# scroll-tech/halo2-snark-aggregator

Measured on AMD Instinct MI355X. Metric: BN254 G1 MSM points/sec, higher is better.
Workload: dtype u32 (9 x 29-bit limbs, Montgomery R = 2^261; 254-bit prime-field integers)

## Files before the change

halo2-snark-aggregator_amd/__init__.py:

```python
from __future__ import annotations

import ctypes as C
import os
from typing import List, Optional, Sequence

_HERE = os.path.dirname(os.path.abspath(__file__))
LIB_PATH = os.path.join(_HERE, "libh2agg.so")
HEADER_PATH = os.path.join(os.path.dirname(_HERE), "include", "h2agg.h")

OK, ERR_INVALID, ERR_DIV_ZERO, ERR_EMPTY, ERR_HIP, ERR_NONCANONICAL, ERR_NOMEM, ERR_BAD_POINT, ERR_PEER, ERR_NOT_IN_TABLE = range(10)
OP_ADD, OP_SUB, OP_MUL, OP_SQR, OP_INV, OP_DIV = range(6)
FR_FFT_LOCAL = 10
FR_FFT_MAX_K = 24
FR_QUOTIENT_MAX_K = 28
LAUNCH_ELEMENTWISE = (8, 256)
LAUNCH_SCALAR_MUL = (16, 32)
LAUNCH_SIZE_ORDER = (4, 256)
LAUNCH_MSM_FIX = (12, 64)
LAUNCH_MSM_BIG = (8, 64)
FR_POLY_CHUNK = 11
FR_SCAN_CHUNK = 11
FR_PROD_MAX_COLUMNS = 16
FR_SORT_TILE = 11
FR_SORT_TILE_MIN = 4
# ... 69 lines not shown
        "h2agg_host_alloc": (i32, [ctxp, sz, C.POINTER(vp)]),
        "h2agg_host_free": (i32, [ctxp, vp]),
        "h2agg_eval_flat": (i32, [ctxp, u8p, u8p, u8p, sz, vp]),
        "h2agg_bases_upload": (i32, [ctxp, u8p, sz, C.POINTER(u64)]),
        "h2agg_bases_generate": (i32, [ctxp, vp, sz, C.POINTER(u64)]),
        "h2agg_bases_precompute": (i32, [ctxp, u64, i32]),
        "h2agg_bases_download": (i32, [ctxp, u64, sz, sz, vp]),
        "h2agg_bases_free": (i32, [ctxp, u64]),
        "h2agg_g1_msm_preloaded": (i32, [ctxp, u64, u8p, sz, vp]),
        "h2agg_instance_commitment": (i32, [ctxp, u64, u8p, sz, sz, vp]),
        "h2agg_g1_msm_device": (i32, [ctxp, u64, vp, sz, vp]),
        "h2agg_g1_msm_device_async": (i32, [ctxp, u64, vp, sz, vp]),
        "h2agg_schema_create": (i32, [ctxp, C.POINTER(C.c_void_p)]),
        "h2agg_schema_destroy": (None, [C.c_void_p]),
        "h2agg_schema_node_commitment": (i32, [C.c_void_p, C.c_char_p, u8p, C.POINTER(C.c_uint32)]),
        "h2agg_schema_node_eval": (i32, [C.c_void_p, u8p, C.POINTER(C.c_uint32)]),
        "h2agg_schema_node_scalar": (i32, [C.c_void_p, u8p, C.POINTER(C.c_uint32)]),
        "h2agg_schema_node_add": (i32, [C.c_void_p, C.c_uint32, C.c_uint32, C.POINTER(C.c_uint32)]),
        "h2agg_schema_node_mul": (i32, [C.c_void_p, C.c_uint32, C.c_uint32, C.POINTER(C.c_uint32)]),
        "h2agg_schema_estimate": (i32, [C.c_void_p, C.c_uint32, C.POINTER(C.c_size_t)]),
        "h2agg_schema_evaluation_queries": (i32, [C.c_void_p, sz, C.POINTER(C.c_char_p), u8p, u8p,
                                                  C.POINTER(C.c_uint32)]),
        "h2agg_schema_batch_multi_open": (i32, [C.c_void_p, C.c_char_p, sz, C.POINTER(C.c_int32), u8p,
                                                C.POINTER(C.c_uint32), sz, u8p, u8p, u8p,
                                                C.POINTER(C.c_uint32), C.POINTER(C.c_uint32)]),
        "h2agg_schema_shplonk_multi_open": (i32, [C.c_void_p, C.c_char_p, sz, C.POINTER(C.c_uint32), C.POINTER(C.c_int32), u8p,
                                                  C.POINTER(C.c_uint32), u8p, u8p, u8p, u8p, u8p,
                                                  C.POINTER(C.c_uint32), C.POINTER(C.c_uint32)]),
        "h2agg_schema_eval": (i32, [C.c_void_p, C.c_uint32, vp, C.POINTER(i32), vp]),
        "h2agg_evaluate_multiopen_proof": (i32, [C.c_void_p, C.c_uint32, C.c_uint32, vp, vp]),
        "h2agg_evaluate_multiopen_prepare": (i32, [C.c_void_p, C.c_uint32, C.c_uint32]),
        "h2agg_schema_name_count": (C.c_size_t, [C.c_void_p]),
        "h2agg_schema_name": (C.c_char_p, [C.c_void_p, C.c_size_t]),
        "h2agg_g1_msm_device_batch_async": (C.c_int, [C.c_void_p, C.c_uint64, C.c_void_p, C.c_size_t, C.c_size_t, C.c_void_p]),
        "h2agg_schema_query_set_commitment": (C.c_int, [C.c_void_p, C.c_uint32, C.c_char_p]),
        "h2agg_g1_batch_to_affine_device": (C.c_int, [C.c_void_p, C.c_void_p, C.c_size_t, C.c_char_p]),
        "h2agg_schema_names_joined": (C.c_size_t, [C.c_void_p, C.c_char_p, C.c_size_t]),
        "h2agg_schema_point_list_len": (C.c_size_t, [C.c_void_p]),
        "h2agg_poseidon_squeeze_batch": (i32, [ctxp, u8p, sz, sz, C.POINTER(C.c_uint32), sz, vp]),
        "h2agg_transcript_read_batch": (i32, [ctxp, u8p, sz, sz, C.c_char_p, sz, u8p, sz, u8p, sz, vp, vp]),
        "h2agg_vk_create": (i32, [ctxp, u8p, sz, C.POINTER(C.c_void_p)]),
        "h2agg_vk_set_transcript": (i32, [C.c_void_p, i32]),
        "h2agg_vk_set_multiopen": (i32, [C.c_void_p, i32]),
        "h2agg_hash_transcript_read_batch": (i32, [ctxp, i32, u8p, sz, sz, C.c_char_p, sz, u8p, sz, u8p, sz, vp, vp]),
        "h2agg_hash_transcript_read_batch_host": (i32, [i32, u8p, sz, sz, C.c_char_p, sz, u8p, sz, u8p, sz, vp, vp, i32]),
        "h2agg_hash_digest_host": (i32, [i32, u8p, sz, vp]),
        "h2agg_vk_destroy": (None, [C.c_void_p]),
        "h2agg_verify_aggregation": (i32, [ctxp, vp, sz, u8p, u8p, vp, vp, vp, C.POINTER(i32)]),
        "h2agg_verify_aggregation_ex": (i32, [ctxp, vp, sz, u8p, u8p, vp, vp, vp, C.POINTER(i32), vp, sz]),
        "h2agg_verify_aggregation_sharded": (i32, [ctxp, vp, sz, vp, u8p, u8p, vp, vp, vp, C.POINTER(i32), vp, sz]),
        "h2agg_debug_configure": (i32, [ctxp, C.c_char_p, i32]),
        "h2agg_debug_lean_variant": (i32, [i32, i32]),
        "h2agg_debug_table_identity": (i32, [ctxp, u64, C.POINTER(i32), C.POINTER(i32)]),
        "h2agg_verify_proofs": (i32, [ctxp, vp, sz, u8p, u8p, vp, vp, C.POINTER(C.c_int32), C.POINTER(i32), vp, sz]),
        "h2agg_verify_plan_stats": (i32, [ctxp, C.POINTER(C.c_uint64), C.POINTER(C.c_uint64), C.POINTER(C.c_uint64)]),
        "h2agg_last_phases": (C.c_char_p, [ctxp]),
        "h2agg_transcript_configure": (i32, [ctxp, i32]),
        "h2agg_poseidon_squeeze_batch_host": (i32, [u8p, sz, sz, C.POINTER(C.c_uint32), sz, vp, i32]),
        "h2agg_host_threads": (i32, []),
        "h2agg_host_sponge_kind": (i32, []),
        "h2agg_comm_unique_id": (i32, [vp]),
        "h2agg_comm_init_rank": (i32, [ctxp, u8p, i32, i32]),
        "h2agg_comm_create": (i32, [C.POINTER(i32), i32, C.POINTER(ctxp)]),
        "h2agg_comm_size": (i32, [ctxp]),
        "h2agg_comm_rank": (i32, [ctxp]),
        "h2agg_comm_last_error": (C.c_char_p, []),
        "h2agg_allgather_add_points": (i32, [C.POINTER(ctxp), i32, u8p, sz, vp]),
        "h2agg_pairing_check": (i32, [ctxp, u8p, u8p, sz, C.POINTER(i32)]),
        "h2agg_g2_batch_decompress": (i32, [ctxp, u8p, sz, vp]),
        "h2agg_bases_fft": (i32, [ctxp, u64, C.c_uint, i32, C.POINTER(u64)]),
        "h2agg_params_setup": (i32, [ctxp, C.c_uint, u8p, C.POINTER(u64), C.POINTER(u64)]),
        "h2agg_fr_fft": (i32, [ctxp, vp, C.c_uint, i32, u8p, vp]),
        "h2agg_fr_fft_device": (i32, [ctxp, vp, C.c_uint, i32, u8p, vp]),
        "h2agg_fr_fft_batch": (i32, [ctxp, vp, C.c_size_t, C.c_uint, i32, u8p, vp]),
        "h2agg_fr_poly_eval": (i32, [ctxp, vp, sz, C.c_uint, C.POINTER(C.c_uint32), sz, u8p, sz, vp]),
        "h2agg_fr_poly_eval_device": (i32, [ctxp, vp, sz, C.c_uint, C.POINTER(C.c_uint32), sz, u8p, sz, vp]),
        "h2agg_fr_poly_divide": (i32, [ctxp, vp, C.c_uint, u8p, vp, vp]),
        "h2agg_fr_poly_divide_device": (i32, [ctxp, vp, C.c_uint, u8p, vp, vp]),
        "h2agg_kzg_multiopen": (i32, [ctxp, u64, vp, sz, C.c_uint, C.POINTER(C.c_uint32), sz, u8p, sz, u8p, vp,
                                      C.POINTER(C.c_uint32), C.POINTER(sz)]),
        "h2agg_kzg_multiopen_device": (i32, [ctxp, u64, vp, sz, C.c_uint, C.POINTER(C.c_uint32), sz, u8p, sz, u8p, vp,
                                             C.POINTER(C.c_uint32), C.POINTER(sz)]),
        "h2agg_kzg_shplonk_begin": (i32, [ctxp, u64, vp, sz, C.c_uint, C.POINTER(C.c_uint32), sz, u8p, sz, u8p, u8p, u8p, vp,
                                          C.POINTER(vp)]),
        "h2agg_kzg_shplonk_finish": (i32, [vp, u8p, vp]),
        "h2agg_kzg_shplonk_destroy": (None, [vp]),
        "h2agg_fr_batch_invert": (i32, [ctxp, vp, sz, vp]),
        "h2agg_fr_batch_invert_device": (i32, [ctxp, vp, sz, vp]),
        "h2agg_fr_grand_product": (i32, [ctxp, vp, vp, C.c_uint, sz, u8p, vp, vp]),
        "h2agg_fr_grand_product_device": (i32, [ctxp, vp, vp, C.c_uint, sz, u8p, vp, vp]),
        "h2agg_permutation_product": (i32, [ctxp, vp, vp, sz, C.c_uint, sz, u8p, u8p, u8p, u8p, u8p, vp, vp]),
        "h2agg_permutation_product_device": (i32, [ctxp, vp, vp, sz, C.c_uint, sz, u8p, u8p, u8p, u8p, u8p, vp, vp]),
        "h2agg_lookup_product": (i32, [ctxp, vp, vp, vp, vp, C.c_uint, sz, u8p, u8p, vp, vp]),
        "h2agg_lookup_product_device": (i32, [ctxp, vp, vp, vp, vp, C.c_uint, sz, u8p, u8p, vp, vp]),
        "h2agg_lookup_permute": (i32, [ctxp, vp, vp, C.c_uint, sz, vp, vp]),
        "h2agg_lookup_permute_device": (i32, [ctxp, vp, vp, C.c_uint, sz, vp, vp]),
        "h2agg_lookup_batch_permute": (i32, [ctxp, vp, vp, sz, C.c_uint, sz, vp, vp, vp]),
        "h2agg_lookup_batch_product": (i32, [ctxp, vp, vp, vp, vp, sz, C.c_uint, sz, u8p, u8p, vp, vp]),
        "h2agg_lookup_store_permute": (i32, [ctxp, u64, sz, u64, sz, sz, sz, u64, sz, u64, sz, vp]),
        "h2agg_lookup_store_product": (i32, [ctxp, u64, sz, u64, sz, u64, sz, u64, sz, sz, sz, u8p, u8p, u64, sz, vp]),
        "h2agg_lookup_configure": (i32, [ctxp, sz]),
        "h2agg_lookup_chunk_rule": (sz, [sz, sz]),
        "h2agg_fr_columns_compress": (i32, [ctxp, vp, sz, C.c_uint, u8p, vp]),
        "h2agg_fr_columns_compress_device": (i32, [ctxp, vp, sz, C.c_uint, u8p, vp]),
        "h2agg_vk_expressions_eval": (i32, [ctxp, vp, i32, sz, C.c_uint, vp, vp, vp, u8p, u8p, vp]),
        "h2agg_vk_expressions_eval_device": (i32, [ctxp, vp, i32, sz, C.c_uint, vp, vp, vp, u8p, u8p, vp]),
# ... 969 lines not shown
        _need(g2_aff, 128 * n, "g2_aff")
        ok = C.c_int()
        self._check(self._lib.h2agg_pairing_check(self._ctx, g1_aff, g2_aff, n, C.byref(ok)))
        return bool(ok.value)

    def pairing_product(self, g1_aff: bytes, g2_aff: bytes) -> bytes:
        n = len(g1_aff) // 64
        _need(g1_aff, 64 * n, "g1_aff")
        _need(g2_aff, 128 * n, "g2_aff")
        out = C.create_string_buffer(384)
        self._check(self._lib.h2agg_pairing_product(self._ctx, g1_aff, g2_aff, n, out))
        return out.raw

    def g2_batch_decompress(self, data: bytes) -> bytes:
        n = len(data) // 64
        _need(data, 64 * n, "data")
        out = C.create_string_buffer(max(128 * n, 1))
        self._check(self._lib.h2agg_g2_batch_decompress(self._ctx, data, n, out))
        return out.raw[:128 * n]

    def final_pair_check(self, left_aff: bytes, right_aff: bytes, s_g2: bytes, g2: bytes) -> bool:
        _need(left_aff, 64, "left_aff")
        _need(right_aff, 64, "right_aff")
        _need(s_g2, 128, "s_g2")
        _need(g2, 128, "g2")
        ok = C.c_int()
        self._check(self._lib.h2agg_final_pair_check(self._ctx, left_aff, right_aff, s_g2, g2, C.byref(ok)))
        return bool(ok.value)

    def g1_msm_device_batch_async(self, handle: int, d_scalars_ptr: int, n: int, batch: int, d_out_ptr: int):
        self._check(self._lib.h2agg_g1_msm_device_batch_async(self._ctx, handle, C.c_void_p(d_scalars_ptr), n, batch,
                                                              C.c_void_p(d_out_ptr)))

    def msm_configure(self, window_bits: int = 0, reduce_segment: int = 0, big_bucket_threshold: int = 0):
        self._check(self._lib.h2agg_msm_configure(self._ctx, window_bits, reduce_segment, big_bucket_threshold))

    def msm_configure_glv(self, mode: int = 0):
        self._check(self._lib.h2agg_msm_configure_glv(self._ctx, mode))

    def msm_configure_lanes_per_bucket(self, lanes: int = 0):
        self._check(self._lib.h2agg_msm_configure_lanes_per_bucket(self._ctx, lanes))

    def msm_configure_sort(self, sub_bits: int = 0, tile: int = 0):
        self._check(self._lib.h2agg_msm_configure_sort(self._ctx, sub_bits, tile))

    def debug_configure(self, key: str, value: int):
        self._check(self._lib.h2agg_debug_configure(self._ctx, key.encode(), int(value)))

    def table_may_hold_identity(self, handle: int) -> bool:
        v = C.c_int32(-1)
        self._check(self._lib.h2agg_debug_table_identity(self._ctx, handle, C.byref(v), None))
        return bool(v.value)

    def last_lean_variant(self) -> int:
        v = C.c_int32(-1)
        self._check(self._lib.h2agg_debug_table_identity(self._ctx, 0, None, C.byref(v)))
        return v.value

    def msm_set_tail_overlap(self, level: int = 2):
        self._check(self._lib.h2agg_msm_set_tail_overlap(self._ctx, int(level)))

    def profile_enable(self, on=True, only_stage: Optional[int] = None):
        mode = (2 + int(only_stage)) if (on and only_stage is not None) else int(bool(on))
        self._check(self._lib.h2agg_profile_enable(self._ctx, mode))

    def profile_reset(self):
        self._check(self._lib.h2agg_profile_reset(self._ctx))

    def profile_stages(self):
        out = {}
        for i in range(self._lib.h2agg_profile_stage_count(self._ctx)):
            ms, cnt = C.c_double(), C.c_uint64()
            self._check(self._lib.h2agg_profile_stage_get(self._ctx, i, C.byref(ms), C.byref(cnt)))
            out[self._lib.h2agg_profile_stage_name(self._ctx, i).decode()] = (ms.value, cnt.value)
        return out


def host_sponge_kind() -> str:
    return "ifma" if load_library().h2agg_host_sponge_kind() == 1 else "scalar"


def poseidon_squeeze_batch_host(elems: bytes, nproofs: int, upto: Sequence[int], max_threads: int = 0,
                                kernel: Optional[str] = None) -> bytes:
    lib = load_library()
    max_threads = (max_threads & 0xffff) | {None: 0, "scalar": 0x10000, "ifma": 0x20000}[kernel]
    nelem = (len(elems) // 32) // max(nproofs, 1)
    _need(elems, 32 * nelem * nproofs, "elems")
    nsq = len(upto)
    arr = (C.c_uint32 * max(nsq, 1))(*upto)
    out = C.create_string_buffer(32 * max(nproofs * nsq, 1))
    rc = lib.h2agg_poseidon_squeeze_batch_host(elems, nproofs, nelem, arr, nsq, out, max_threads)
    if rc != OK:
        raise H2AggError(rc, "h2agg_poseidon_squeeze_batch_host: " + ("element >= r" if rc == ERR_NONCANONICAL else "invalid arguments"))
    return out.raw[:32 * nproofs * nsq]


TRANSCRIPT_KINDS = {"poseidon": 0, "sha256": 1, "keccak256": 2}


def _hash_transcript_args(kind, proofs, script, consts, ext_points_aff):
    nproofs = len(proofs)
    plen = 64 * script.count("P") + 32 * script.count("S")
    for p in proofs:
        _need(p, plen, "proof")
    npts, nsq, nx = script.count("P"), script.count("Q"), script.count("X")
    _need(consts, 32 * script.count("C"), "consts")
# ... 213 lines not shown
```

halo2-snark-aggregator_amd/csrc/config_api.inc:

```

namespace {

struct DebugKey {
    const char* name;
    int h2agg_ctx::*field;
    int lo = 1, hi = 0;
    bool zero_ok = false;
};
const DebugKey DEBUG_KEYS[] = {
    {"pcie_slices", &h2agg_ctx::dbg_pcie_slices},
    {"pcie_glv", &h2agg_ctx::dbg_pcie_glv},
    {"pcie_chain", &h2agg_ctx::dbg_pcie_chain},
    {"comb_msm", &h2agg_ctx::dbg_comb_msm},
    {"plan_cache", &h2agg_ctx::dbg_plan_cache},
    {"small_sort", &h2agg_ctx::dbg_small_sort},
    {"eval_split", &h2agg_ctx::dbg_eval_split},
    {"lean_acc", &h2agg_ctx::dbg_lean_acc},
    {"lean_full", &h2agg_ctx::dbg_lean_full},
    {"pre_big", &h2agg_ctx::dbg_pre_big},
    {"tape_lds", &h2agg_ctx::dbg_tape_lds},
    {"prewake", &h2agg_ctx::dbg_prewake},
    {"phases", &h2agg_ctx::dbg_phases},
    {"shard_fail", &h2agg_ctx::dbg_shard_fail},
    {"seg_chunk", &h2agg_ctx::dbg_seg_chunk},
// ... 43 lines not shown
    if (!c) return H2AGG_ERR_INVALID;
    if (lanes != 0 && lanes != 1 && lanes != 2 && lanes != 4 && lanes != 8 && lanes != 16)
        return fail(c, H2AGG_ERR_INVALID, "lanes must be 0, 1, 2, 4, 8 or 16");
    c->cfg_lpb = lanes;
    return H2AGG_OK;
} API_CATCH

int h2agg_msm_configure_sort(h2agg_ctx* c, int sub_bits, int tile) try {
    if (!c) return H2AGG_ERR_INVALID;
    if (sub_bits != 0 && (sub_bits < 4 || sub_bits > SORT_MAX_SUB_BITS))
        return fail(c, H2AGG_ERR_INVALID, "sub_bits must be 0 or in [4, 12]");
    if (tile != 0 && tile != -1 && tile != -2 && tile != -3 && (tile < BLOCK || tile > (1 << 16)))
        return fail(c, H2AGG_ERR_INVALID, "tile must be 0, -1, -2 or in [256, 65536]");
    c->cfg_sub_bits = sub_bits;
    c->cfg_no_stage = tile == -1;
    c->cfg_no_dm = tile == -3;
    c->cfg_stage_l1 = tile == -2;
    c->cfg_tile = tile > 0 ? tile : 0;
    return H2AGG_OK;
} API_CATCH

int h2agg_debug_configure(h2agg_ctx* c, const char* key, int value) try {
    if (!c || !key) return H2AGG_ERR_INVALID;
    const std::string k(key);
    const DebugKey* row = nullptr;
    for (const DebugKey& r : DEBUG_KEYS)
        if (k == r.name) row = &r;
    if (!row) return fail(c, H2AGG_ERR_INVALID, "h2agg_debug_configure: unknown key " + k);
    if (!debug_key_takes(*row, value)) return fail(c, H2AGG_ERR_INVALID, debug_key_range(*row));
#ifndef H2AGG_MEASURE_KNOBS
    if (k == "lean_acc" && value != 1)
        return fail(c, H2AGG_ERR_INVALID, "h2agg_debug_configure: the generic accumulation kernel is in the measure build only (build_ext.py --measure)");
#endif
    if (k == "tape_lds" && c->dbg_tape_lds != value) agg_plans_release(c);
    c->*(row->field) = value;
    return H2AGG_OK;
} API_CATCH

int h2agg_debug_lean_variant(int table_no_identity, int plan_glv) {
    return msm_lean_variant(table_no_identity != 0, plan_glv != 0);
}

int h2agg_debug_table_identity(h2agg_ctx* c, uint64_t handle, int* may_hold_out, int* last_variant_out) try {
    TRY(bind(c));
    if (may_hold_out) {
        Table* t = nullptr;
        TRY(find_table(c, handle, &t));
        *may_hold_out = t->no_identity ? 0 : 1;
    }
    if (last_variant_out) *last_variant_out = c->last_lean_variant;
    return H2AGG_OK;
} API_CATCH

int h2agg_msm_set_tail_overlap(h2agg_ctx* c, int enable) try {
    TRY(bind(c));
    TRY(join_tails(c));
    HIP_TRY(c, hipStreamSynchronize(c->stream));
    c->tail_overlap = enable != 0;
    if (enable >= 1 && enable <= 3) c->overlap_level = enable;
    return H2AGG_OK;
} API_CATCH

int h2agg_profile_enable(h2agg_ctx* c, int enable) try {
    TRY(bind(c));
    if (enable && !c->prof_events_created) {
        for (int r = 0; r < h2agg_ctx::PROF_RING; ++r)
            for (int s = 0; s < ST_N; ++s)
                for (int k = 0; k < 2; ++k) HIP_TRY(c, c->prof[r].ev[s][k].create(EV_TIME_FLAGS));
        c->prof_events_created = true;
    }
    if (!enable) profile_harvest_all(c);
    c->profiling = enable != 0;
    c->prof_only = (enable >= 2 && enable - 2 < ST_N) ? enable - 2 : -1;
    return H2AGG_OK;
} API_CATCH
int h2agg_profile_reset(h2agg_ctx* c) try {
    if (!c) return H2AGG_ERR_INVALID;
    profile_harvest_all(c);
    for (int s = 0; s < ST_N; ++s) {
        c->stage_ms[s] = 0;
        c->stage_launches[s] = 0;
    }
    return H2AGG_OK;
} API_CATCH
int h2agg_profile_stage_count(h2agg_ctx*) { return ST_N; }
const char* h2agg_profile_stage_name(h2agg_ctx*, int i) { return (i >= 0 && i < ST_N) ? STAGE_NAMES[i] : ""; }
int h2agg_profile_stage_get(h2agg_ctx* c, int i, double* total_ms, uint64_t* launches) try {
    if (!c || i < 0 || i >= ST_N) return H2AGG_ERR_INVALID;
    profile_harvest_all(c);
    if (total_ms) *total_ms = c->stage_ms[i];
    if (launches) *launches = c->stage_launches[i];
    return H2AGG_OK;
} API_CATCH

}
```

halo2-snark-aggregator_amd/csrc/sort_kernels.hpp:

```cpp
#pragma once
#include "batch_kernels.hpp"

namespace h2agg {

#ifndef H2AGG_NO_SORT_SETPRIO
#define SORT_PRIO() __builtin_amdgcn_s_setprio(3)
#else
#define SORT_PRIO() ((void)0)
#endif

constexpr int SORT_MAX_PW = 2048;
constexpr int SORT_SUB_BITS = 9;
constexpr int SORT_MAX_SUB_BITS = 12;
constexpr int SORT_MAX_SB = 1 << SORT_MAX_SUB_BITS;
constexpr int SIZE_BINS = 1024;

struct SortPlan {
    int sub_bits;
    uint32_t SB;
    uint32_t ppw;
    uint32_t PW;
    uint32_t tile;
    bool glv;
    uint32_t n_base = 0;
// ... 797 lines not shown
    return x;
}
FP_INLINE void dm_block_scan(uint32_t* v, uint32_t cnt) {
    __syncthreads();
    if (threadIdx.x < 64) {
        const uint32_t lane = threadIdx.x;
        uint32_t x[8], sum = 0;
#pragma unroll
        for (int j = 0; j < 8; ++j) {
            x[j] = (8 * lane + j < cnt) ? v[8 * lane + j] : 0u;
            sum += x[j];
        }
        const uint32_t inc = dm_wave_scan_incl(sum, lane);
        uint32_t off = inc - sum;
#pragma unroll
        for (int j = 0; j < 8; ++j) {
            if (8 * lane + j < cnt) v[8 * lane + j] = off;
            off += x[j];
        }
        if (lane == 63) v[cnt] = inc;
    }
    __syncthreads();
}

__global__ void __launch_bounds__(1024) k_dm_scan(const uint32_t* __restrict__ in, uint32_t n, uint32_t* __restrict__ out) {
    SORT_PRIO();
    __shared__ uint32_t wsum[16];
    const uint32_t tid = threadIdx.x, lane = tid & 63, wave = tid >> 6;
    uint32_t x[8], sum = 0;
#pragma unroll
    for (int j = 0; j < 8; ++j) {
        x[j] = (8 * tid + j < n) ? in[8 * tid + j] : 0u;
        sum += x[j];
    }
    const uint32_t inc = dm_wave_scan_incl(sum, lane);
    if (lane == 63) wsum[wave] = inc;
    __syncthreads();
    uint32_t base = 0;
    for (uint32_t k = 0; k < wave; ++k) base += wsum[k];
    uint32_t off = base + inc - sum;
#pragma unroll
    for (int j = 0; j < 8; ++j) {
        if (8 * tid + j <= n) out[8 * tid + j] = off;
        off += x[j];
    }
    if (8 * tid + 8 == n) out[n] = off;
}

template <bool WIDE>
__global__ void __launch_bounds__(DM_TB1) k_dm_partition(const uint16_t* __restrict__ codes, DmPlan dp,
                                                         uint32_t* __restrict__ pcount, uint32_t* __restrict__ toff,
                                                         uint32_t* __restrict__ items) {
    SORT_PRIO();
    __shared__ uint32_t cnt[DM_MAX_PPW + 1];
    __shared__ __attribute__((aligned(16))) uint32_t stage[DM_T1];
    const uint32_t tile = blockIdx.x, w = blockIdx.y;
    const int tid = threadIdx.x;
    for (uint32_t p = tid; p <= dp.ppw; p += DM_TB1) cnt[p] = 0;
    __syncthreads();
    const size_t row = (size_t)w * dp.n_pad;
    const uint32_t t0 = tile * DM_T1;
    constexpr int G = 8, NV = DM_PER1 / G;
    uint4 v[NV];
    uint32_t sg[NV], zr[NV];
#pragma unroll
    for (int k = 0; k < NV; ++k) {
        const uint32_t i0 = t0 + (k * DM_TB1 + tid) * G;
        sg[k] = 0;
        zr[k] = 0xffu;
        if (WIDE) {
            v[k] = make_uint4(0, 0, 0, 0);
            if (i0 < dp.n_pad) {
                const uint8_t* fl = dm17_flags(codes, dp.n_pad);
                const size_t rb = dp.n_pad >> 3;
                v[k] = *reinterpret_cast<const uint4*>(codes + row + i0);
                sg[k] = fl[(size_t)w * rb + (i0 >> 3)];
                zr[k] = fl[(size_t)(DM17_W + w) * rb + (i0 >> 3)];
            }
        } else {
            v[k] = (i0 < dp.n_pad) ? *reinterpret_cast<const uint4*>(codes + row + i0)
                                   : make_uint4(0x80008000u, 0x80008000u, 0x80008000u, 0x80008000u);
        }
    }
    auto decode = [&](int k, int e, uint32_t& bkt, uint32_t& neg) -> bool {
        const uint32_t wd[4] = {v[k].x, v[k].y, v[k].z, v[k].w};
        const uint32_t code = (wd[e >> 1] >> (16 * (e & 1))) & 0xffffu;
        if (WIDE) {
            bkt = code;
            neg = (sg[k] >> e) & 1u;
            return !((zr[k] >> e) & 1u);
        }
        neg = code >> 15;
        bkt = neg ? (code & 0x7fffu) - 1u : code;
        return code != DM_ZERO;
    };
    uint32_t pr[DM_PER1];
    const uint32_t submask = dp.SB - 1u;
#pragma unroll
    for (int k = 0; k < NV; ++k) {
#pragma unroll
        for (int e = 0; e < G; ++e) {
            uint32_t bkt, neg;
            const uint32_t i = t0 + (k * DM_TB1 + tid) * G + e;
            const bool ok = decode(k, e, bkt, neg) && i < dp.n;
            const uint32_t p = bkt >> dp.sub_bits;
            pr[k * G + e] = ok ? ((p << 16) | atomicAdd(&cnt[p], 1u)) : 0xffffffffu;
        }
    }
    __syncthreads();
    for (uint32_t p = tid; p < dp.ppw; p += DM_TB1) {
        const uint32_t c = cnt[p];
        if (c) atomicAdd(&pcount[w * dp.ppw + p], c);
    }
    dm_block_scan(cnt, dp.ppw);
    uint32_t* tt = toff + ((size_t)w * dp.ntile + tile) * (dp.ppw + 1);
    for (uint32_t p = tid; p <= dp.ppw; p += DM_TB1) tt[p] = cnt[p];
#pragma unroll
    for (int k = 0; k < NV; ++k) {
#pragma unroll
        for (int e = 0; e < G; ++e) {
            const uint32_t q = pr[k * G + e];
            if (q == 0xffffffffu) continue;
            uint32_t bkt, neg;
            decode(k, e, bkt, neg);
            const uint32_t i = t0 + (k * DM_TB1 + tid) * G + e;
            stage[cnt[q >> 16] + (q & 0xffffu)] = ((bkt & submask) << (dp.idx_bits + 1)) | (neg << dp.idx_bits) | i;
        }
    }
    __syncthreads();
    const uint32_t total = cnt[dp.ppw];
    uint32_t* out = items + (size_t)w * dp.n_row + t0;
    for (uint32_t k = 4 * tid; k < total; k += 4 * DM_TB1)
        *reinterpret_cast<uint4*>(out + k) = *reinterpret_cast<const uint4*>(stage + k);
}

FP_INLINE uint32_t dm_entry(uint32_t it, const DmPlan& dp, uint32_t idxmask) {
    uint32_t idx = it & idxmask;
    uint32_t e = ((it >> dp.idx_bits) & 1u) << 31;
    if (idx >= dp.n_pts) {
        idx -= dp.n_pts;
        e |= ENT_ENDO;
    }
    return e | idx;
}

typedef __attribute__((address_space(3))) uint32_t lds_u32;
FP_INLINE uint32_t dm_wave_agg_add(lds_u32* h, uint32_t b, bool valid) {
    const uint32_t lane = __lane_id();
    uint64_t todo = __ballot(valid);
    uint32_t res = 0;
    bool pending = valid;
#pragma unroll 1
    for (int round = 0; round < 2 && todo; ++round) {
        const int lead = __ffsll((unsigned long long)todo) - 1;
        const uint32_t bl = __shfl(b, lead);
        const bool mine = pending && b == bl;
        const uint64_t same = __ballot(mine);
        uint32_t base = 0;
        if ((int)lane == lead)
            base = __hip_atomic_fetch_add(&h[bl], (uint32_t)__popcll(same), __ATOMIC_RELAXED, __HIP_MEMORY_SCOPE_WORKGROUP);
        base = __shfl(base, lead);
        if (mine) {
            res = base + (uint32_t)__popcll(same & ((1ull << lane) - 1ull));
            pending = false;
        }
        todo &= ~same;
    }
    if (pending) res = __hip_atomic_fetch_add(&h[b], 1u, __ATOMIC_RELAXED, __HIP_MEMORY_SCOPE_WORKGROUP);
    return res;
}

template <bool PLACE>
__device__ __attribute__((noinline)) void dm_long_pass(const uint32_t* __restrict__ rowp, const lds_u32* rstart,
                                                       const lds_u32* rpre, lds_u32* h, uint32_t* __restrict__ out,
                                                       uint32_t ntile, int idx_bits, uint32_t n_pts) {
    constexpr int LB = 8;
    const uint32_t lane = threadIdx.x & 63u, wv = threadIdx.x >> 6;
    const int sh = idx_bits + 1;
    const uint32_t idxmask = (1u << idx_bits) - 1u;
    for (uint32_t t = wv; t < ntile; t += DM_TB2 / 64) {
        const uint32_t len = rpre[t + 1] - rpre[t];
        const uint32_t* src = rowp + (size_t)t * DM_T1 + rstart[t];
        for (uint32_t k0 = 0; k0 < len; k0 += 64 * LB) {
            uint32_t v[LB];
#pragma unroll
            for (int j = 0; j < LB; ++j) {
                const uint32_t k = k0 + j * 64 + lane;
                v[j] = k < len ? src[k] : 0u;
            }
#pragma unroll
            for (int j = 0; j < LB; ++j) {
                const bool ok = k0 + j * 64 + lane < len;
                const uint32_t at = dm_wave_agg_add(h, v[j] >> sh, ok);
                if (PLACE && ok) {
                    uint32_t idx = v[j] & idxmask, e = ((v[j] >> idx_bits) & 1u) << 31;
                    if (idx >= n_pts) {
                        idx -= n_pts;
                        e |= ENT_ENDO;
                    }
                    out[at] = e | idx;
                }
            }
        }
    }
}

template <int PER>
__global__ void __launch_bounds__(DM_TB2) __attribute__((amdgpu_waves_per_eu(6, 6))) k_dm_bucket_sort(const uint32_t* __restrict__ pstart,
                                                           const uint32_t* __restrict__ toff,
                                                           const uint32_t* __restrict__ items, DmPlan dp, uint32_t NB,
                                                           uint32_t* __restrict__ hist, uint32_t* __restrict__ offs,
                                                           uint32_t* __restrict__ entries) {
    SORT_PRIO();
    constexpr int TB = DM_TB2;
    __shared__ uint32_t h[DM_MAX_PPW + 8];
    __shared__ uint32_t rstart[DM_MAX_TILES];
    __shared__ uint32_t rpre[DM_MAX_TILES + 8];
    constexpr int DM_STAGE = PER * DM_TB2;
    __shared__ __attribute__((aligned(16))) uint32_t stage[DM_STAGE];
    const uint32_t p = gridDim.x - 1u - blockIdx.x, w = p / dp.ppw, pl = p - w * dp.ppw;
    const int tid = threadIdx.x;
    const uint32_t start = pstart[p], total = pstart[p + 1] - start;
    for (uint32_t b = tid; b <= dp.SB; b += TB) h[b] = 0;
    for (uint32_t t = tid; t < dp.ntile; t += TB) {
        const uint32_t* tt = toff + ((size_t)w * dp.ntile + t) * (dp.ppw + 1) + pl;
        const uint32_t a = tt[0];
        rstart[t] = a;
        rpre[t] = tt[1] - a;
    }
    dm_block_scan(rpre, dp.ntile);
    const uint32_t* rowp = items + (size_t)w * dp.n_row;
    const int sh = dp.idx_bits + 1;
    const uint32_t idxmask = (1u << dp.idx_bits) - 1u;
    const uint32_t key0 = w * NB + (pl << dp.sub_bits);
    const float guess = total ? (float)dp.ntile / (float)total : 0.f;
    auto locate = [&](uint32_t k) -> const uint32_t* {
        uint32_t t = (uint32_t)((float)k * guess);
        if (t >= dp.ntile) t = dp.ntile - 1;
        while (rpre[t] > k) --t;
        while (rpre[t + 1] <= k) ++t;
        return rowp + (size_t)t * DM_T1 + rstart[t] + (k - rpre[t]);
    };
    if (total <= (uint32_t)DM_STAGE) {
        uint32_t it[PER], rk[PER];
#pragma unroll
        for (int j = 0; j < PER; ++j) {
            const uint32_t k = tid + j * TB;
            it[j] = k < total ? *locate(k) : 0u;
        }
#pragma unroll
        for (int j = 0; j < PER; ++j) {
            const uint32_t k = tid + j * TB;
            rk[j] = k < total ? atomicAdd(&h[it[j] >> sh], 1u) : 0u;
        }
        __syncthreads();
        for (uint32_t b = tid; b < dp.SB; b += TB) hist[key0 + b] = h[b];
        dm_block_scan(h, dp.SB);
        for (uint32_t b = tid; b < dp.SB; b += TB) offs[key0 + b] = start + h[b];
#pragma unroll
        for (int j = 0; j < PER; ++j) {
            const uint32_t k = tid + j * TB;
            if (k < total) stage[h[it[j] >> sh] + rk[j]] = dm_entry(it[j], dp, idxmask);
        }
        __syncthreads();
        for (uint32_t k = tid; k < total; k += TB) entries[start + k] = stage[k];
        return;
    }
    if (total <= 8u * (uint32_t)DM_STAGE) {
        constexpr int MB = 4;
        for (uint32_t k0 = tid; k0 < total; k0 += MB * TB) {
            uint32_t v[MB];
#pragma unroll
            for (int j = 0; j < MB; ++j) v[j] = k0 + j * TB < total ? *locate(k0 + j * TB) : 0u;
#pragma unroll
            for (int j = 0; j < MB; ++j)
                if (k0 + j * TB < total) atomicAdd(&h[v[j] >> sh], 1u);
        }
        __syncthreads();
        for (uint32_t b = tid; b < dp.SB; b += TB) hist[key0 + b] = h[b];
        dm_block_scan(h, dp.SB);
        for (uint32_t b = tid; b < dp.SB; b += TB) offs[key0 + b] = start + h[b];
        __syncthreads();
        for (uint32_t k0 = tid; k0 < total; k0 += MB * TB) {
            uint32_t v[MB];
#pragma unroll
            for (int j = 0; j < MB; ++j) v[j] = k0 + j * TB < total ? *locate(k0 + j * TB) : 0u;
#pragma unroll
            for (int j = 0; j < MB; ++j)
                if (k0 + j * TB < total) entries[start + atomicAdd(&h[v[j] >> sh], 1u)] = dm_entry(v[j], dp, idxmask);
        }
        return;
    }
    dm_long_pass<false>(rowp, (const lds_u32*)rstart, (const lds_u32*)rpre, (lds_u32*)h, nullptr, dp.ntile, dp.idx_bits, dp.n_pts);
    __syncthreads();
    for (uint32_t b = tid; b < dp.SB; b += TB) hist[key0 + b] = h[b];
    dm_block_scan(h, dp.SB);
    for (uint32_t b = tid; b < dp.SB; b += TB) offs[key0 + b] = start + h[b];
    __syncthreads();
    dm_long_pass<true>(rowp, (const lds_u32*)rstart, (const lds_u32*)rpre, (lds_u32*)h, entries + start, dp.ntile, dp.idx_bits, dp.n_pts);
}

FP_INLINE uint32_t size_bin(uint32_t len) { return (SIZE_BINS - 1) - (len < SIZE_BINS ? len : SIZE_BINS - 1); }

__global__ void __launch_bounds__(BLOCK) k_size_count(const uint32_t* __restrict__ hist, uint32_t nbt,
                                                      uint32_t* __restrict__ bin_count) {
    SORT_PRIO();
    __shared__ uint32_t cnt[SIZE_BINS];
    for (uint32_t b = threadIdx.x; b < SIZE_BINS; b += BLOCK) cnt[b] = 0;
    __syncthreads();
    for (uint32_t k = blockIdx.x * BLOCK + threadIdx.x; k < nbt; k += gridDim.x * BLOCK)
        atomicAdd(&cnt[size_bin(hist[k])], 1u);
    __syncthreads();
    for (uint32_t b = threadIdx.x; b < SIZE_BINS; b += BLOCK)
        if (cnt[b]) atomicAdd(&bin_count[b], cnt[b]);
}
__global__ void __launch_bounds__(BLOCK) k_size_scatter(const uint32_t* __restrict__ hist, uint32_t nbt,
                                                        uint32_t* __restrict__ bin_cursor, uint32_t* __restrict__ order) {
    SORT_PRIO();
    __shared__ uint32_t cnt[SIZE_BINS];
    __shared__ uint32_t baseb[SIZE_BINS];
    for (uint32_t b = threadIdx.x; b < SIZE_BINS; b += BLOCK) cnt[b] = 0;
    __syncthreads();
    for (uint32_t k = blockIdx.x * BLOCK + threadIdx.x; k < nbt; k += gridDim.x * BLOCK)
        atomicAdd(&cnt[size_bin(hist[k])], 1u);
    __syncthreads();
    for (uint32_t b = threadIdx.x; b < SIZE_BINS; b += BLOCK) {
        const uint32_t v = cnt[b];
        baseb[b] = v ? atomicAdd(&bin_cursor[b], v) : 0u;
        cnt[b] = 0;
    }
    __syncthreads();
    for (uint32_t k = blockIdx.x * BLOCK + threadIdx.x; k < nbt; k += gridDim.x * BLOCK) {
        const uint32_t b = size_bin(hist[k]);
        order[baseb[b] + atomicAdd(&cnt[b], 1u)] = k;
    }
}

}
```

include/h2agg.h:

```cpp
#ifndef H2AGG_H
#define H2AGG_H

#include <stddef.h>
#include <stdint.h>

#ifdef __cplusplus
extern "C" {
#endif

typedef struct h2agg_ctx h2agg_ctx;

enum {
    H2AGG_OK = 0,
    H2AGG_ERR_INVALID = 1,
    H2AGG_ERR_DIV_ZERO = 2,
    H2AGG_ERR_EMPTY = 3,
    H2AGG_ERR_HIP = 4,
    H2AGG_ERR_NONCANONICAL = 5,
    H2AGG_ERR_NOMEM = 6,
    H2AGG_ERR_BAD_POINT = 7,
    H2AGG_ERR_PEER = 8,
    H2AGG_ERR_NOT_IN_TABLE = 9
};

// ... 262 lines not shown

int h2agg_columns_create(h2agg_ctx* ctx, size_t m, unsigned k, uint64_t* handle_out);
int h2agg_columns_destroy(h2agg_ctx* ctx, uint64_t handle);
int h2agg_columns_info(h2agg_ctx* ctx, uint64_t handle, size_t* m_out, unsigned* k_out);
int h2agg_columns_write(h2agg_ctx* ctx, uint64_t handle, size_t first, size_t count, const uint8_t* host);
int h2agg_columns_read(h2agg_ctx* ctx, uint64_t handle, size_t first, size_t count, uint8_t* host);
int h2agg_columns_ptr(h2agg_ctx* ctx, uint64_t handle, size_t first, void** d_ptr_out);
int h2agg_columns_move(h2agg_ctx* ctx, uint64_t src, size_t sfirst, uint64_t dst, size_t dfirst, size_t count, int32_t rotation);
int h2agg_columns_fft(h2agg_ctx* ctx, uint64_t src, size_t sfirst, uint64_t dst, size_t dfirst, size_t count, int inverse,
                      const uint8_t shift[32]);
int h2agg_columns_commit(h2agg_ctx* ctx, uint64_t bases_handle, uint64_t src, size_t first, size_t count, uint8_t* out_aff);
int h2agg_columns_sigmas(h2agg_ctx* ctx, const uint32_t* mapping, size_t m, unsigned k, size_t usable, const uint8_t delta[32],
                         uint64_t dst_lagrange, size_t lfirst, uint64_t dst_coeff, size_t cfirst);
int h2agg_columns_witness_check(h2agg_ctx* ctx, const h2agg_vk* vk, unsigned what, uint64_t advice, size_t afirst, uint64_t fixed,
                                size_t ffirst, uint64_t instance, size_t ifirst, const uint8_t* challenges, const uint8_t theta[32],
                                const uint32_t* mapping, size_t max_rows, uint32_t* counts, uint32_t* first_rows, uint32_t* rows,
                                uint64_t* total);
int h2agg_columns_shplonk_begin(h2agg_ctx* ctx, uint64_t g_handle, uint64_t src, size_t first, size_t npoly, const uint32_t* queries,
                                size_t nq, const uint8_t* points, size_t npoints, const uint8_t* evals, const uint8_t y[32],
                                const uint8_t v[32], uint8_t h1_aff[64], h2agg_shplonk** out);

#define H2AGG_PK_COSETS 1u
#define H2AGG_PK_FIXED_LAGRANGE 0
#define H2AGG_PK_SIGMA_LAGRANGE 1
#define H2AGG_PK_FIXED_COEFF 2
#define H2AGG_PK_SIGMA_COEFF 3
#define H2AGG_PK_LAGRANGE_COEFF 4
#define H2AGG_PK_COSET 5
typedef struct h2agg_pk h2agg_pk;
int h2agg_pk_create(h2agg_ctx* ctx, const h2agg_vk* vk, const uint8_t* fixed, const uint8_t* sigma, unsigned forms, h2agg_pk** out);
int h2agg_pk_create_resident(h2agg_ctx* ctx, const h2agg_vk* vk, const void* d_fixed, const void* d_sigma, unsigned forms,
                             h2agg_pk** out);
int h2agg_pk_bytes(const h2agg_vk* vk, unsigned forms, size_t* bytes_out);
int h2agg_pk_info(const h2agg_pk* pk, unsigned* k_out, unsigned* e_out, size_t* fixed_out, size_t* sigma_out, unsigned* forms_out,
                  size_t* bytes_out);
int h2agg_pk_ptr(const h2agg_pk* pk, int which, size_t coset, const void** d_ptr_out, size_t* columns_out);
int h2agg_pk_quotient(h2agg_ctx* ctx, const h2agg_pk* pk, const void* d_advice, const void* d_instance, const void* d_perm_z,
                      const void* d_lookup_z, const void* d_lookup_ap, const void* d_lookup_sp, const uint8_t* challenges,
                      const uint8_t theta[32], const uint8_t beta[32], const uint8_t gamma[32], const uint8_t y[32],
                      const uint8_t delta[32], void* d_h);
int h2agg_pk_quotient_work_bytes(const h2agg_pk* pk, size_t* bytes_out);
void h2agg_pk_destroy(h2agg_pk* pk);

int h2agg_fr_tape_eval(h2agg_ctx* ctx, const uint8_t* consts, size_t nconst, const uint32_t* ops3, size_t nops,
                       const uint32_t* out_regs, size_t nout, uint8_t* out);

int h2agg_msm_configure(h2agg_ctx* ctx, int window_bits, int reduce_segment, int big_bucket_threshold);
int h2agg_msm_configure_glv(h2agg_ctx* ctx, int mode);
int h2agg_msm_configure_lanes_per_bucket(h2agg_ctx* ctx, int lanes);
int h2agg_msm_configure_sort(h2agg_ctx* ctx, int sub_bits, int tile);
int h2agg_debug_configure(h2agg_ctx* ctx, const char* key, int value);
int h2agg_debug_lean_variant(int table_no_identity, int plan_glv);
int h2agg_debug_table_identity(h2agg_ctx* ctx, uint64_t handle, int* may_hold_out, int* last_variant_out);
int h2agg_msm_set_tail_overlap(h2agg_ctx* ctx, int enable);
int h2agg_profile_enable(h2agg_ctx* ctx, int enable);
int h2agg_profile_reset(h2agg_ctx* ctx);
int h2agg_profile_stage_count(h2agg_ctx* ctx);
const char* h2agg_profile_stage_name(h2agg_ctx* ctx, int i);
int h2agg_profile_stage_get(h2agg_ctx* ctx, int i, double* total_ms, uint64_t* launches);

#ifdef __cplusplus
}
#endif
#endif
```

Baseline: 831.4 million.

## Rework MSM bucket sort: branch-free code decode and run-chunked trip table

```diff
diff --git a/halo2-snark-aggregator_amd/__init__.py b/halo2-snark-aggregator_amd/__init__.py
--- a/halo2-snark-aggregator_amd/__init__.py
+++ b/halo2-snark-aggregator_amd/__init__.py
@@ -145,6 +145,7 @@
         "h2agg_debug_configure": (i32, [ctxp, C.c_char_p, i32]),
         "h2agg_debug_lean_variant": (i32, [i32, i32]),
         "h2agg_debug_table_identity": (i32, [ctxp, u64, C.POINTER(i32), C.POINTER(i32)]),
+        "h2agg_debug_sort_readback": (i32, [ctxp, i32, vp, sz]),
         "h2agg_verify_proofs": (i32, [ctxp, vp, sz, u8p, u8p, vp, vp, C.POINTER(C.c_int32), C.POINTER(i32), vp, sz]),
         "h2agg_verify_plan_stats": (i32, [ctxp, C.POINTER(C.c_uint64), C.POINTER(C.c_uint64), C.POINTER(C.c_uint64)]),
         "h2agg_last_phases": (C.c_char_p, [ctxp]),
@@ -1220,6 +1221,12 @@
         self._check(self._lib.h2agg_debug_table_identity(self._ctx, handle, C.byref(v), None))
         return bool(v.value)
 
+    def sort_readback(self, which: int, words: int):
+        import numpy as np
+        out = np.empty(int(words), dtype=np.uint32)
+        self._check(self._lib.h2agg_debug_sort_readback(self._ctx, which, out.ctypes.data, int(words)))
+        return out
+
     def last_lean_variant(self) -> int:
         v = C.c_int32(-1)
         self._check(self._lib.h2agg_debug_table_identity(self._ctx, 0, None, C.byref(v)))
diff --git a/halo2-snark-aggregator_amd/csrc/config_api.inc b/halo2-snark-aggregator_amd/csrc/config_api.inc
--- a/halo2-snark-aggregator_amd/csrc/config_api.inc
+++ b/halo2-snark-aggregator_amd/csrc/config_api.inc
@@ -119,6 +119,17 @@
     return H2AGG_OK;
 } API_CATCH
 
+int h2agg_debug_sort_readback(h2agg_ctx* c, int which, uint32_t* out, size_t words) try {
+    TRY(bind(c));
+    if (!out || which < 0 || which > 2) return fail(c, H2AGG_ERR_INVALID, "h2agg_debug_sort_readback: which must be 0 (hist), 1 (offs) or 2 (entries)");
+    TRY(join_tails(c));
+    HIP_TRY(c, hipStreamSynchronize(c->stream));
+    const auto& b = which == 0 ? c->hist[0] : which == 1 ? c->offs[0] : c->entries[0];
+    if (!b.p || words * 4 > b.cap) return fail(c, H2AGG_ERR_INVALID, "h2agg_debug_sort_readback: the array holds fewer words");
+    HIP_TRY(c, hipMemcpy(out, b.p, words * 4, hipMemcpyDeviceToHost));
+    return H2AGG_OK;
+} API_CATCH
+
 int h2agg_msm_set_tail_overlap(h2agg_ctx* c, int enable) try {
     TRY(bind(c));
     TRY(join_tails(c));
diff --git a/halo2-snark-aggregator_amd/csrc/sort_kernels.hpp b/halo2-snark-aggregator_amd/csrc/sort_kernels.hpp
--- a/halo2-snark-aggregator_amd/csrc/sort_kernels.hpp
+++ b/halo2-snark-aggregator_amd/csrc/sort_kernels.hpp
@@ -873,79 +873,103 @@
                                                          uint32_t* __restrict__ pcount, uint32_t* __restrict__ toff,
                                                          uint32_t* __restrict__ items) {
     SORT_PRIO();
+    static_assert(DM_MAX_PPW == DM_TB1, "a counter per thread");
     __shared__ uint32_t cnt[DM_MAX_PPW + 1];
     __shared__ __attribute__((aligned(16))) uint32_t stage[DM_T1];
     const uint32_t tile = blockIdx.x, w = blockIdx.y;
     const int tid = threadIdx.x;
-    for (uint32_t p = tid; p <= dp.ppw; p += DM_TB1) cnt[p] = 0;
+    cnt[tid] = 0;
+    if (tid == 0) cnt[DM_MAX_PPW] = 0;
     __syncthreads();
     const size_t row = (size_t)w * dp.n_pad;
     const uint32_t t0 = tile * DM_T1;
     constexpr int G = 8, NV = DM_PER1 / G;
-    uint4 v[NV];
+    uint32_t v[NV][4];
     uint32_t sg[NV], zr[NV];
 #pragma unroll
     for (int k = 0; k < NV; ++k) {
         const uint32_t i0 = t0 + (k * DM_TB1 + tid) * G;
+        uint4 q = make_uint4(0x80008000u, 0x80008000u, 0x80008000u, 0x80008000u);
         sg[k] = 0;
         zr[k] = 0xffu;
-        if (WIDE) {
-            v[k] = make_uint4(0, 0, 0, 0);
-            if (i0 < dp.n_pad) {
+        if (i0 < dp.n_pad) {
+            q = *reinterpret_cast<const uint4*>(codes + row + i0);
+            if (WIDE) {
                 const uint8_t* fl = dm17_flags(codes, dp.n_pad);
                 const size_t rb = dp.n_pad >> 3;
-                v[k] = *reinterpret_cast<const uint4*>(codes + row + i0);
                 sg[k] = fl[(size_t)w * rb + (i0 >> 3)];
                 zr[k] = fl[(size_t)(DM17_W + w) * rb + (i0 >> 3)];
             }
+        }
+        v[k][0] = q.x, v[k][1] = q.y, v[k][2] = q.z, v[k][3] = q.w;
+        if (i0 + G > dp.n) {
+            const uint32_t keep = i0 < dp.n ? dp.n - i0 : 0u;
+            if (WIDE) {
+                zr[k] |= 0xffu << keep;
+            } else {
+#pragma unroll
+                for (int d = 0; d < 4; ++d) {
+                    const uint32_t gone = (2u * d >= keep ? 0xffffu : 0u) | (2u * d + 1u >= keep ? 0xffff0000u : 0u);
+                    v[k][d] = (v[k][d] & ~gone) | (0x80008000u & gone);
+                }
+            }
+        }
+    }
+    auto decode2 = [](uint32_t wd, uint32_t& r, uint32_t& ng) {
+        ng = (wd >> 15) & 0x00010001u;
+        r = ((wd & 0x7fff7fffu) | 0x80008000u) - ng;
+    };
+    const int sb = dp.sub_bits;
+    const uint32_t ppw = dp.ppw;
+    uint32_t so[DM_PER1], rank[DM_PER1];
+#pragma unroll
+    for (int k = 0; k < NV; ++k) {
+        if (WIDE) {
+#pragma unroll
+            for (int e = 0; e < G; ++e) {
+                const uint32_t code = (v[k][e >> 1] >> (16 * (e & 1))) & 0xffffu;
+                so[k * G + e] = ((zr[k] >> e) & 1u) ? ppw : code >> sb;
+            }
         } else {
-            v[k] = (i0 < dp.n_pad) ? *reinterpret_cast<const uint4*>(codes + row + i0)
-                                   : make_uint4(0x80008000u, 0x80008000u, 0x80008000u, 0x80008000u);
-        }
-    }
-    auto decode = [&](int k, int e, uint32_t& bkt, uint32_t& neg) -> bool {
-        const uint32_t wd[4] = {v[k].x, v[k].y, v[k].z, v[k].w};
-        const uint32_t code = (wd[e >> 1] >> (16 * (e & 1))) & 0xffffu;
-        if (WIDE) {
-            bkt = code;
-            neg = (sg[k] >> e) & 1u;
-            return !((zr[k] >> e) & 1u);
-        }
-        neg = code >> 15;
-        bkt = neg ? (code & 0x7fffu) - 1u : code;
-        return code != DM_ZERO;
-    };
-    uint32_t pr[DM_PER1];
-    const uint32_t submask = dp.SB - 1u;
-#pragma unroll
-    for (int k = 0; k < NV; ++k) {
-#pragma unroll
-        for (int e = 0; e < G; ++e) {
-            uint32_t bkt, neg;
-            const uint32_t i = t0 + (k * DM_TB1 + tid) * G + e;
-            const bool ok = decode(k, e, bkt, neg) && i < dp.n;
-            const uint32_t p = bkt >> dp.sub_bits;
-            pr[k * G + e] = ok ? ((p << 16) | atomicAdd(&cnt[p], 1u)) : 0xffffffffu;
-        }
-    }
-    __syncthreads();
-    for (uint32_t p = tid; p < dp.ppw; p += DM_TB1) {
-        const uint32_t c = cnt[p];
-        if (c) atomicAdd(&pcount[w * dp.ppw + p], c);
+#pragma unroll
+            for (int d = 0; d < 4; ++d) {
+                uint32_t r, ng;
+                decode2(v[k][d], r, ng);
+                so[k * G + 2 * d] = min(((r & 0xffffu) >> sb) - ppw, ppw);
+                so[k * G + 2 * d + 1] = min((r >> (16 + sb)) - ppw, ppw);
+            }
+        }
+#pragma unroll
+        for (int e = 0; e < G; ++e) rank[k * G + e] = atomicAdd(&cnt[so[k * G + e]], 1u);
+    }
+    __syncthreads();
+    if ((uint32_t)tid < dp.ppw) {
+        const uint32_t c = cnt[tid];
+        if (c) atomicAdd(&pcount[w * dp.ppw + tid], c);
     }
     dm_block_scan(cnt, dp.ppw);
     uint32_t* tt = toff + ((size_t)w * dp.ntile + tile) * (dp.ppw + 1);
-    for (uint32_t p = tid; p <= dp.ppw; p += DM_TB1) tt[p] = cnt[p];
+    if ((uint32_t)tid < dp.ppw) tt[tid] = cnt[tid];
+    if (tid == 0) tt[dp.ppw] = cnt[dp.ppw];
+    const uint32_t submask = dp.SB - 1u;
 #pragma unroll
     for (int k = 0; k < NV; ++k) {
+        const uint32_t i0 = t0 + (k * DM_TB1 + tid) * G;
+        uint32_t at[G];
+#pragma unroll
+        for (int e = 0; e < G; ++e) at[e] = cnt[so[k * G + e]];
 #pragma unroll
         for (int e = 0; e < G; ++e) {
-            const uint32_t q = pr[k * G + e];
-            if (q == 0xffffffffu) continue;
-            uint32_t bkt, neg;
-            decode(k, e, bkt, neg);
-            const uint32_t i = t0 + (k * DM_TB1 + tid) * G + e;
-            stage[cnt[q >> 16] + (q & 0xffffu)] = ((bkt & submask) << (dp.idx_bits + 1)) | (neg << dp.idx_bits) | i;
+            uint32_t x;
+            if (WIDE) {
+                const uint32_t code = (v[k][e >> 1] >> (16 * (e & 1))) & 0xffffu;
+                x = ((code & submask) << 1) | ((sg[k] >> e) & 1u);
+            } else {
+                uint32_t r, ng;
+                decode2(v[k][e >> 1], r, ng);
+                x = (e & 1) ? ((r >> 15) & ~1u) | (ng >> 16) : (r << 1) | ng;
+            }
+            stage[at[e] + rank[k * G + e]] = (x << dp.idx_bits) | i0 | (uint32_t)e;
         }
     }
     __syncthreads();
@@ -1026,6 +1050,11 @@
     }
 }
 
+constexpr int DM_G = 16;
+constexpr int DM_NG = DM_TB2 / DM_G;
+constexpr int DM_TRIP_SH = 22;
+static_assert(DM_MAX_TILES * DM_T1 <= (1 << DM_TRIP_SH) && DM_G <= (1 << (32 - DM_TRIP_SH)), "trip word");
+static_assert(DM_MAX_TILES <= DM_TB2 && DM_MAX_PPW <= DM_TB2, "one thread per run, one per bucket of the partition");
 template <int PER>
 __global__ void __launch_bounds__(DM_TB2) __attribute__((amdgpu_waves_per_eu(6, 6))) k_dm_bucket_sort(const uint32_t* __restrict__ pstart,
                                                            const uint32_t* __restrict__ toff,
@@ -1038,87 +1067,121 @@
     __shared__ uint32_t rstart[DM_MAX_TILES];
     __shared__ uint32_t rpre[DM_MAX_TILES + 8];
     constexpr int DM_STAGE = PER * DM_TB2;
+    constexpr int MB = 4;
+    static_assert(8 * DM_STAGE / DM_G + DM_MAX_TILES + MB * DM_NG <= DM_STAGE && PER * DM_NG <= DM_STAGE, "trip table");
     __shared__ __attribute__((aligned(16))) uint32_t stage[DM_STAGE];
     const uint32_t p = gridDim.x - 1u - blockIdx.x, w = p / dp.ppw, pl = p - w * dp.ppw;
     const int tid = threadIdx.x;
     const uint32_t start = pstart[p], total = pstart[p + 1] - start;
+    const bool skew = total > 8u * (uint32_t)DM_STAGE;
     for (uint32_t b = tid; b <= dp.SB; b += TB) h[b] = 0;
-    for (uint32_t t = tid; t < dp.ntile; t += TB) {
-        const uint32_t* tt = toff + ((size_t)w * dp.ntile + t) * (dp.ppw + 1) + pl;
-        const uint32_t a = tt[0];
-        rstart[t] = a;
-        rpre[t] = tt[1] - a;
+    uint32_t ra = 0, rlen = 0;
+    if ((uint32_t)tid < dp.ntile) {
+        const uint32_t* tt = toff + ((size_t)w * dp.ntile + tid) * (dp.ppw + 1) + pl;
+        ra = tt[0];
+        rlen = tt[1] - ra;
+        rstart[tid] = ra;
+        rpre[tid] = skew ? rlen : (rlen + DM_G - 1) / DM_G;
     }
     dm_block_scan(rpre, dp.ntile);
     const uint32_t* rowp = items + (size_t)w * dp.n_row;
     const int sh = dp.idx_bits + 1;
     const uint32_t idxmask = (1u << dp.idx_bits) - 1u;
     const uint32_t key0 = w * NB + (pl << dp.sub_bits);
-    const float guess = total ? (float)dp.ntile / (float)total : 0.f;
-    auto locate = [&](uint32_t k) -> const uint32_t* {
-        uint32_t t = (uint32_t)((float)k * guess);
-        if (t >= dp.ntile) t = dp.ntile - 1;
-        while (rpre[t] > k) --t;
-        while (rpre[t + 1] <= k) ++t;
-        return rowp + (size_t)t * DM_T1 + rstart[t] + (k - rpre[t]);
-    };
-    if (total <= (uint32_t)DM_STAGE) {
-        uint32_t it[PER], rk[PER];
+    if (skew) {
+        dm_long_pass<false>(rowp, (const lds_u32*)rstart, (const lds_u32*)rpre, (lds_u32*)h, nullptr, dp.ntile, dp.idx_bits, dp.n_pts);
+        __syncthreads();
+        if ((uint32_t)tid < dp.SB) hist[key0 + tid] = h[tid];
+        dm_block_scan(h, dp.SB);
+        if ((uint32_t)tid < dp.SB) offs[key0 + tid] = start + h[tid];
+        __syncthreads();
+        dm_long_pass<true>(rowp, (const lds_u32*)rstart, (const lds_u32*)rpre, (lds_u32*)h, entries + start, dp.ntile, dp.idx_bits, dp.n_pts);
+        return;
+    }
+    uint32_t* trips = stage;
+    const uint32_t ntrip = __builtin_amdgcn_readfirstlane(rpre[dp.ntile]);
+    if ((uint32_t)tid < dp.ntile) {
+        uint32_t q = rpre[tid], src = (uint32_t)tid * DM_T1 + ra;
+        for (uint32_t left = rlen; left; ++q, src += DM_G) {
+            const uint32_t c = left < (uint32_t)DM_G ? left : (uint32_t)DM_G;
+            trips[q] = ((c - 1u) << DM_TRIP_SH) | src;
+            left -= c;
+        }
+    }
+    __syncthreads();
+    const uint32_t grp = (uint32_t)tid / DM_G, li = (uint32_t)tid % DM_G;
+    constexpr uint32_t SRC = (1u << DM_TRIP_SH) - 1u;
+    if (total <= (uint32_t)DM_STAGE && ntrip <= (uint32_t)(PER * DM_NG)) {
+        const uint32_t g0 = __builtin_amdgcn_readfirstlane(grp);
+        const uint32_t nj = ntrip > g0 ? (ntrip - g0 + DM_NG - 1) / DM_NG : 0u;
+        uint32_t it[PER], rk[PER], have = 0;
+#pragma unroll
+        for (int j0 = 0; j0 < PER; j0 += 8) {
+            uint32_t e[8];
+#pragma unroll
+            for (int j = 0; j < 8; ++j) e[j] = trips[(j0 + j) * DM_NG + grp];
+#pragma unroll
+            for (int j = 0; j < 8; ++j) {
+                it[j0 + j] = 0;
+                if ((uint32_t)(j0 + j) < nj && (j0 + j) * DM_NG + grp < ntrip && li <= (e[j] >> DM_TRIP_SH)) {
+                    it[j0 + j] = rowp[(e[j] & SRC) + li];
+                    have |= 1u << (j0 + j);
+                }
+            }
+        }
 #pragma unroll
         for (int j = 0; j < PER; ++j) {
-            const uint32_t k = tid + j * TB;
-            it[j] = k < total ? *locate(k) : 0u;
-        }
+            rk[j] = 0;
+            if ((uint32_t)j < nj && ((have >> j) & 1u)) rk[j] = atomicAdd(&h[it[j] >> sh], 1u);
+        }
+        __syncthreads();
+        if ((uint32_t)tid < dp.SB) hist[key0 + tid] = h[tid];
+        dm_block_scan(h, dp.SB);
+        if ((uint32_t)tid < dp.SB) offs[key0 + tid] = start + h[tid];
 #pragma unroll
         for (int j = 0; j < PER; ++j) {
-            const uint32_t k = tid + j * TB;
-            rk[j] = k < total ? atomicAdd(&h[it[j] >> sh], 1u) : 0u;
-        }
-        __syncthreads();
-        for (uint32_t b = tid; b < dp.SB; b += TB) hist[key0 + b] = h[b];
-        dm_block_scan(h, dp.SB);
-        for (uint32_t b = tid; b < dp.SB; b += TB) offs[key0 + b] = start + h[b];
-#pragma unroll
-        for (int j = 0; j < PER; ++j) {
-            const uint32_t k = tid + j * TB;
-            if (k < total) stage[h[it[j] >> sh] + rk[j]] = dm_entry(it[j], dp, idxmask);
-        }
-        __syncthreads();
-        for (uint32_t k = tid; k < total; k += TB) entries[start + k] = stage[k];
+            if ((uint32_t)j < nj && ((have >> j) & 1u)) stage[h[it[j] >> sh] + rk[j]] = dm_entry(it[j], dp, idxmask);
+        }
+        __syncthreads();
+        uint32_t* dst = entries + start;
+#pragma unroll
+        for (int j = 0; j < PER; ++j)
+            if (tid + j * TB < (int)total) dst[tid + j * TB] = stage[tid + j * TB];
         return;
     }
-    if (total <= 8u * (uint32_t)DM_STAGE) {
-        constexpr int MB = 4;
-        for (uint32_t k0 = tid; k0 < total; k0 += MB * TB) {
-            uint32_t v[MB];
-#pragma unroll
-            for (int j = 0; j < MB; ++j) v[j] = k0 + j * TB < total ? *locate(k0 + j * TB) : 0u;
-#pragma unroll
-            for (int j = 0; j < MB; ++j)
-                if (k0 + j * TB < total) atomicAdd(&h[v[j] >> sh], 1u);
-        }
-        __syncthreads();
-        for (uint32_t b = tid; b < dp.SB; b += TB) hist[key0 + b] = h[b];
-        dm_block_scan(h, dp.SB);
-        for (uint32_t b = tid; b < dp.SB; b += TB) offs[key0 + b] = start + h[b];
-        __syncthreads();
-        for (uint32_t k0 = tid; k0 < total; k0 += MB * TB) {
-            uint32_t v[MB];
-#pragma unroll
-            for (int j = 0; j < MB; ++j) v[j] = k0 + j * TB < total ? *locate(k0 + j * TB) : 0u;
-#pragma unroll
-            for (int j = 0; j < MB; ++j)
-                if (k0 + j * TB < total) entries[start + atomicAdd(&h[v[j] >> sh], 1u)] = dm_entry(v[j], dp, idxmask);
-        }
-        return;
-    }
-    dm_long_pass<false>(rowp, (const lds_u32*)rstart, (const lds_u32*)rpre, (lds_u32*)h, nullptr, dp.ntile, dp.idx_bits, dp.n_pts);
-    __syncthreads();
-    for (uint32_t b = tid; b < dp.SB; b += TB) hist[key0 + b] = h[b];
+    for (uint32_t q0 = grp; q0 < ntrip; q0 += MB * DM_NG) {
+        uint32_t v[MB];
+        bool ok[MB];
+#pragma unroll
+        for (int j = 0; j < MB; ++j) {
+            const uint32_t q = q0 + j * DM_NG;
+            const uint32_t e = trips[q];
+            ok[j] = q < ntrip && li <= (e >> DM_TRIP_SH);
+            v[j] = ok[j] ? rowp[(e & SRC) + li] : 0u;
+        }
+#pragma unroll
+        for (int j = 0; j < MB; ++j)
+            if (ok[j]) atomicAdd(&h[v[j] >> sh], 1u);
+    }
+    __syncthreads();
+    if ((uint32_t)tid < dp.SB) hist[key0 + tid] = h[tid];
     dm_block_scan(h, dp.SB);
-    for (uint32_t b = tid; b < dp.SB; b += TB) offs[key0 + b] = start + h[b];
-    __syncthreads();
-    dm_long_pass<true>(rowp, (const lds_u32*)rstart, (const lds_u32*)rpre, (lds_u32*)h, entries + start, dp.ntile, dp.idx_bits, dp.n_pts);
+    if ((uint32_t)tid < dp.SB) offs[key0 + tid] = start + h[tid];
+    __syncthreads();
+    for (uint32_t q0 = grp; q0 < ntrip; q0 += MB * DM_NG) {
+        uint32_t v[MB];
+        bool ok[MB];
+#pragma unroll
+        for (int j = 0; j < MB; ++j) {
+            const uint32_t q = q0 + j * DM_NG;
+            const uint32_t e = trips[q];
+            ok[j] = q < ntrip && li <= (e >> DM_TRIP_SH);
+            v[j] = ok[j] ? rowp[(e & SRC) + li] : 0u;
+        }
+#pragma unroll
+        for (int j = 0; j < MB; ++j)
+            if (ok[j]) entries[start + atomicAdd(&h[v[j] >> sh], 1u)] = dm_entry(v[j], dp, idxmask);
+    }
 }
 
 FP_INLINE uint32_t size_bin(uint32_t len) { return (SIZE_BINS - 1) - (len < SIZE_BINS ? len : SIZE_BINS - 1); }
diff --git a/include/h2agg.h b/include/h2agg.h
--- a/include/h2agg.h
+++ b/include/h2agg.h
@@ -338,6 +338,7 @@
 int h2agg_debug_configure(h2agg_ctx* ctx, const char* key, int value);
 int h2agg_debug_lean_variant(int table_no_identity, int plan_glv);
 int h2agg_debug_table_identity(h2agg_ctx* ctx, uint64_t handle, int* may_hold_out, int* last_variant_out);
+int h2agg_debug_sort_readback(h2agg_ctx* ctx, int which, uint32_t* out, size_t words);
 int h2agg_msm_set_tail_overlap(h2agg_ctx* ctx, int enable);
 int h2agg_profile_enable(h2agg_ctx* ctx, int enable);
 int h2agg_profile_reset(h2agg_ctx* ctx);
```

New measurement: 835.1 million, median of 3. No clear change (+0.4%).
